# tennisonliu/bayesian-neural-network

Measured on AMD Instinct MI355X. Metric: MC-forward-samples/sec + KL-elements/sec, 784-1200-1200-10 BNN, higher is better.
Workload: dtype bf16

## Files before the change

### bayesian-neural-network_amd/bnn_hip/engine.py

```python
from __future__ import annotations

import os
from typing import List, Optional, Sequence, Tuple

import torch

from . import _lib as L
from . import ops
from .functional import AllReduceSumFn, BBBLinearFn, ElboFn, LayerCall, LRLinearFn, NetCall, NLLFn
from .ops import Predictive
from .runtime import state, take_samples


CAST_INPUT_MIN_SAMPLES = 4
CAST_INPUT_MIN_SAMPLES_LR = 1
LR_SQUARES_MIN_SAMPLES = 7
SPLIT_MIN_SAMPLES = 4
SPLIT_MIN_WEIGHTS = 250_000
SPLIT_MAX_UNITS = 1024

FUSED_ELBO_NODE = True


FINAL_ROWS_MAX_SAMPLES = 16
# ... 464 lines not shown
                self.ws[i] = ops.sample_workspace(S, sp.in_out[0], sp.in_out[1], dev)
        shared0 = self.lr and not self.G > 1 and lr_unit_samples(S, True) == 1
        k3s_first = (self.lr and hid == torch.bfloat16 and len(self.specs) > 1 and self.specs[0].in_out[0] % 8 == 0 and
                     lr_use_split(self.specs[0].in_out[1], S, B, shared0) and not self.G > 1)
        shared0 = shared0 and k3s_first
        self.x16 = (torch.empty(self.x.shape, dtype=torch.bfloat16, device=dev)
                    if (hid == torch.bfloat16 and self.x.dtype == torch.float32 and
                        (self.lib[0] or S >= (CAST_INPUT_MIN_SAMPLES_LR if self.lr else CAST_INPUT_MIN_SAMPLES)) and
                        not k3s_first) else None)
        self.x16_lo = torch.empty(self.x.shape, dtype=torch.bfloat16, device=dev) if (self.x3 and self.x16 is not None) else None
        self.lr_sq = self.lr and (self.x16 is not None or (k3s_first and hid == torch.bfloat16)) and S >= LR_SQUARES_MIN_SAMPLES
        self.x16_sq = torch.empty(self.x.shape, dtype=torch.bfloat16, device=dev) if (self.lr_sq and self.x16 is not None) else None
        self.bufs_sq = [torch.empty(b.shape, dtype=torch.bfloat16, device=dev)
                        if (self.lr_sq and i < len(self.bufs) - 1 and b.dtype == torch.bfloat16) else None for i, b in enumerate(self.bufs)]
        self.split = [ops.split_scratch(S, B, sp.in_out[1], dev)
                      if (not self.lr and hid == torch.bfloat16 and not self.lib[i] and
                          use_split(sp.in_out[0], sp.in_out[1], S, B)) else None
                      for i, sp in enumerate(self.specs)]
        self.lr_split = [ops.lr_split_scratch(lr_unit_samples(S, shared0 and i == 0), B, sp.in_out[1], dev)
                         if (self.lr and hid == torch.bfloat16 and i < len(self.specs) - 1 and
                             lr_use_split(sp.in_out[1], S, B, shared0 and i == 0)) else None
                         for i, sp in enumerate(self.specs)]
        self.wsigma = [torch.empty_like(sp.m.weight_rho.detach())
                      if (not self.lr and hid == torch.bfloat16 and not lb and hoist_sigma(*sp.in_out, S, B)) else None
                      for sp, lb in zip(self.specs, self.lib)]
        self.wfrag = [None] * len(self.specs)
        if self.lr_sq:
            frag_bytes = L.load().bnn_lr_prepare_x3_bytes if self.lr_x3 else L.load().bnn_lr_prepare_bytes
            self.wfrag = [torch.empty(frag_bytes(*sp.in_out) // 4, dtype=torch.float32, device=dev)
                          if (lr_use_prepare(sp.in_out[1], S, B) and not (shared0 and i == 0) and not (self.lr_x3 and i == nl_ - 1)) else None
                          for i, sp in enumerate(self.specs)]
        nl = len(self.specs)
        self.lr_rider = None
        if (self.lr_sq and not self.lr_x3 and self.wfrag[nl - 1] is None and any(w is not None for w in self.wfrag) and
                self.scratch is not None and not wide_nll(self.specs, B) and self.specs[-1].in_out[1] <= 16 and S <= LR_FINAL_ROWS_MAX_SAMPLES):
            self.wfrag[nl - 1] = torch.empty(L.load().bnn_lr_prepare_bytes(*self.specs[-1].in_out) // 4, dtype=torch.float32, device=dev)
        if (self.lr and hid == torch.bfloat16 and nl > 1 and self.wfrag[nl - 1] is None and self.scratch is not None and
                not wide_nll(self.specs, B) and self.specs[-1].in_out[1] <= 16 and S <= 16 and self.lr_split[nl - 2] is not None and
                lr_kslice_expected(*self.specs[-2].in_out, S, B)):
            sp = self.specs[-1]
            self.lr_rider = dict(w_mu=sp.m.weight_mu.detach(), w_rho=sp.m.weight_rho.detach(), b_mu=sp.m.bias_mu.detach(),
                                 b_rho=sp.m.bias_rho.detach(), workspace=self.ws[nl - 1],
                                 w_frag=torch.empty(L.load().bnn_lr_prepare_bytes(*sp.in_out) // 4, dtype=torch.float32, device=dev))
        self.pre_from = presample_from(self.specs, S, B, hid)
        self.rows = self.pre_from >= 0
        self.w_pre, self.b_pre = [None] * len(self.specs), [None] * len(self.specs)
        if self.rows:
            for i in range(self.pre_from + 1, len(self.specs)):
                k_i, n_i = self.specs[i].in_out
                self.w_pre[i] = torch.empty((S, n_i, k_i), dtype=torch.bfloat16, device=dev)
                self.b_pre[i] = torch.empty((S, n_i), dtype=torch.float32, device=dev)
                self.ws[i] = ops.sample_workspace(S, k_i, n_i, dev)
        self.k1b2 = self._k1b2_layers() if state.pieces else [False] * nl
        for i in range(nl - 1):
            if self.k1b2[i] and i == 0 and self.x16 is not None:
                self.x16 = ops.pieces_activation(self.x.shape, dev)
            elif self.k1b2[i] and i > 0 and self.k1b2[i - 1]:
                self.bufs[i - 1] = ops.pieces_activation(self.bufs[i - 1].shape, dev)
        self.wpieces = [ops.param_pieces(sp.in_out[1], sp.in_out[0], dev) if (k and state.param_pieces) else None
                        for sp, k in zip(self.specs, self.k1b2)]
        for w, pc in zip(self.wsigma, self.wpieces):
            if pc is not None:
                w.bnn_param_pieces = pc
        self.graph = None
        self.calls = None
        if capture == "calls":
            rec_stream = self.stream if self.stream is not None else torch.cuda.current_stream()
            with torch.cuda.stream(rec_stream):
                self._enqueue()
            take_samples(self.total_samples)
            torch.cuda.synchronize()
            before = torch.cuda.memory_stats(dev).get("allocation.all.allocated", 0)
            with L.recording() as calls, torch.cuda.stream(rec_stream):
                self._eager()
            take_samples(self.total_samples * self.per_replay)
            torch.cuda.synchronize()
            if torch.cuda.memory_stats(dev).get("allocation.all.allocated", 0) != before:
                raise ops.BnnHipError("GraphedElbo(capture='calls'): the evaluation allocated device memory while it was recorded -- "
                                      "a replay would launch on freed buffers; use capture=True (hipGraph) for this configuration")
            self.calls = list(calls)
        elif capture:
            self._enqueue()
            take_samples(self.total_samples)
            torch.cuda.synchronize()
            side = self.stream if self.stream is not None else torch.cuda.Stream()
            side.wait_stream(torch.cuda.current_stream())
            with torch.cuda.stream(side):
                g = torch.cuda.CUDAGraph()
                with torch.cuda.graph(g, stream=side):
                    self._eager()
            torch.cuda.current_stream().wait_stream(side)
            self.graph = g

    def _enqueue(self):
        math_mode = self.math
        h_sq, h_lo = None, None
        hoist = [i for i, w in enumerate(self.wsigma) if w is not None]
        h = self.x
        if self.x16 is not None or hoist:
            ops.eval_prepare([self.specs[i].m.weight_rho.detach() for i in hoist], [self.wsigma[i] for i in hoist],
                             cast=self.x if self.x16 is not None else None, cast_out=self.x16,
                             cast_out_sq=self.x16_sq, cast_out_lo=self.x16_lo,
                             mus=[self.specs[i].m.weight_mu.detach() for i in hoist], pieces=[self.wpieces[i] for i in hoist])
            if self.x16 is not None:
                h, h_sq, h_lo = self.x16, self.x16_sq, self.x16_lo
        last = len(self.specs) - 1
        if self.lr and any(w is not None for w in self.wfrag):
            jobs = [dict(w_mu=sp.m.weight_mu.detach(), w_rho=sp.m.weight_rho.detach(), b_mu=sp.m.bias_mu.detach(),
                         b_rho=sp.m.bias_rho.detach(), workspace=self.ws[i], out=self.wfrag[i])
                    for i, sp in enumerate(self.specs) if self.wfrag[i] is not None]
            ops.lr_prepare_many(jobs, x3=self.lr_x3)
# ... 26 lines not shown
                if i == last:
                    ops.elbo_finalize(workspaces=self.ws, logits=self.bufs[i], **fin_kw)
            else:
                kw = self._bbb_kw(i, h, h_lo, common)
                if i == last and self.rows:
                    ops.bbb_final_fwd((h, None, None, None, None),
                                      dict(n_samples=self.n_local, prior=sp.m._prior_spec, math_mode=math_mode, relu=sp.relu,
                                           y_dtype=self.bufs[i].dtype, eps_mode=L.EPS_ZERO, want_stats=False, out=self.bufs[i],
                                           w_sampled=self.w_pre[i], b_sampled=self.b_pre[i]),
                                      dict(workspaces=self.ws, **fin_kw))
                elif i == last:
                    ops.bbb_final_fwd((h,) + p, kw, dict(workspaces=self.ws[:last], **fin_kw))
                else:
                    ops.bbb_linear_fwd(h, *p, **kw)
            h, h_lo = self.bufs[i], self.bufs_lo[i]
        if self.lr:
            ops.elbo_finalize(workspaces=self.ws, logits=h, **fin_kw)

    def _common_kw(self, i):
        sp = self.specs[i]
        grp = dict(sample_group=self.group, sample_group_stride=self.samples) if self.G > 1 else {}
        return dict(n_samples=self.n_local, math_mode=self.math, relu=sp.relu, y_dtype=self.bufs[i].dtype,
                    eps_mode=L.EPS_PHILOX, seed=state.seed, layer_id=sp.layer_id, sample_offset=self.lo,
                    sample_counter=self.counter, workspace=self.ws[i], out=self.bufs[i], form=state.form, **grp)

    def _bbb_kw(self, i, h, h_lo, common):
        sp = self.specs[i]
        kw = dict(prior=sp.m._prior_spec, want_stats=True, split_scratch=self.split[i], w_sigma=self.wsigma[i], **common)
        if self.x3:
            kw.update(x_lo=h_lo if h.dtype == torch.bfloat16 else None, out_lo=self.bufs_lo[i])
        if i == self.pre_from and i < len(self.specs) - 1:
            grp = dict(sample_group=self.group, sample_group_stride=self.samples) if self.G > 1 else {}
            kw["rider"] = ops.build_sample_job(
                [dict(w_mu=q.m.weight_mu.detach(), w_rho=q.m.weight_rho.detach(), b_mu=q.m.bias_mu.detach(),
                      b_rho=q.m.bias_rho.detach(), prior=q.m._prior_spec, layer_id=q.layer_id,
                      workspace=self.ws[j], w_out=self.w_pre[j], b_out=self.b_pre[j])
                 for j, q in enumerate(self.specs) if j > i],
                n_samples=self.n_local, seed=state.seed, sample_offset=self.lo, sample_counter=self.counter, **grp)
        return kw

    def _k1b2_layers(self):
        res = [False] * len(self.specs)
        if self.lr or self.math != L.MATH_BF16:
            return res
        h = self.x16 if self.x16 is not None else self.x
        for i, sp in enumerate(self.specs[:-1]):
            if not self.lib[i] and self.wsigma[i] is not None and h.dtype == torch.bfloat16:
                p = tuple(t.detach() for t in (sp.m.weight_mu, sp.m.weight_rho, sp.m.bias_mu, sp.m.bias_rho))
                plan = ops.bbb_plan(h, *p, **self._bbb_kw(i, h, None, self._common_kw(i)))
                res[i] = plan["form"] == L.FORM_GEMM and plan["waves"] == 8
            h = self.bufs[i]
        return res

    def _sample_layer(self, i, grp):
        sp = self.specs[i]
        p = tuple(t.detach() for t in (sp.m.weight_mu, sp.m.weight_rho, sp.m.bias_mu, sp.m.bias_rho))
        ops.bbb_sample_weights([dict(w_mu=p[0], w_rho=p[1], b_mu=p[2], b_rho=p[3], prior=sp.m._prior_spec, layer_id=sp.layer_id,
                                     workspace=self.ws[i], w_out=self.lib_w[i], b_out=self.lib_b[i])],
                               n_samples=self.n_local, seed=state.seed, sample_offset=self.lo, sample_counter=self.counter, **grp)

    def _eager(self):
        for _ in range(self.per_replay):
            self._enqueue()

    def replay(self) -> torch.Tensor:
        if self.calls is not None:
            for fn, args, name in self.calls:
                rc = fn(*args)
                if rc:
                    L.check(rc, name)
            take_samples(self.total_samples * self.per_replay)
            return self.sums
        if self.stream is not None:
            with torch.cuda.stream(self.stream):
                self.graph.replay() if self.graph is not None else self._eager()
        elif self.graph is not None:
            self.graph.replay()
        else:
            self._eager()
        take_samples(self.total_samples * self.per_replay)
        return self.sums

    @property
    def logits(self) -> torch.Tensor:
        return self.bufs[-1]


class GraphedPredict(GraphedElbo):

    def __init__(self, net, x: torch.Tensor, samples: int, capture: bool = True, stream: Optional[torch.cuda.Stream] = None):
        if net.mode != "classification":
            raise ops.BnnHipError("GraphedPredict: the MC-averaged class prediction exists for classification networks")
        xf = net._flat(x)
        self.probs = torch.empty((xf.shape[0], net._specs()[-1].in_out[1]), dtype=torch.float32, device=x.device)
        self.preds = torch.empty(xf.shape[0], dtype=torch.int64, device=x.device)
        super().__init__(net, x, torch.zeros(xf.shape[0], dtype=torch.int64, device=x.device), samples, capture=capture, stream=stream)

    def _enqueue(self):
        super()._enqueue()
        ops.mc_softmax_mean(self.logits, 1.0 / self.samples, out_probs=self.probs, out_preds=self.preds if self.world == 1 else None,
                            want_preds=self.world == 1)

    def replay(self):
        super().replay()
        if self.world > 1:
            import torch.distributed as dist
# ... 92 lines not shown
```

### bayesian-neural-network_amd/bnn_hip/ops.py

```python
from __future__ import annotations

import ctypes as C
import math
from dataclasses import dataclass
from typing import NamedTuple, Optional, Sequence

import torch

from . import _lib as L
from ._lib import BnnHipError


@dataclass(frozen=True)
class PriorSpec:
    mixture: bool = False
    sigma_p: float = 1.0
    pi: float = 0.5
    sigma1: float = 1.0
    sigma2: float = 1.0

    @staticmethod
    def from_init(prior_init: Sequence[float], mixture: bool) -> "PriorSpec":
        if mixture:
            assert len(prior_init) == 3, "Scale Mixture Prior requires three values in prior initialisation"
# ... 20 lines not shown

def _f32c(t: torch.Tensor, name: str) -> torch.Tensor:
    if t.dtype != torch.float32:
        raise BnnHipError(f"{name} must be float32, got {t.dtype}")
    return t if t.is_contiguous() else t.contiguous()


def _ptr(t: Optional[torch.Tensor]) -> Optional[int]:
    return None if t is None else t.data_ptr()


def _dt(t: torch.Tensor) -> int:
    if t.dtype == torch.float32:
        return L.F32
    if t.dtype == torch.bfloat16:
        return L.BF16
    raise BnnHipError(f"activations must be float32 or bfloat16, got {t.dtype}")


def _exact_unless_bf16(math_mode: int) -> int:
    return L.MATH_F32 if math_mode == L.MATH_BF16X3 else math_mode


def pieces_activation(shape, device) -> torch.Tensor:
    shape = tuple(int(d) for d in shape)
    if len(shape) not in (2, 3) or min(shape) < 1:
        raise BnnHipError(f"pieces_activation: shape must be [batch,features] or [rows,batch,features], got {shape}")
    rows = shape[0] if len(shape) == 3 else 1
    t = torch.zeros((rows * ((shape[-2] + 127) // 128), (shape[-1] + 31) // 32, 8, 64, 8), dtype=torch.bfloat16, device=device)
    t.bnn_pieces = shape
    return t


def param_pieces(out_features: int, in_features: int, device) -> torch.Tensor:
    return torch.zeros(((out_features + 15) // 16, (in_features + 31) // 32, 4, 64, 4), dtype=torch.float32, device=device)


def pieces_shape(t: Optional[torch.Tensor]):
    return getattr(t, "bnn_pieces", None) if t is not None else None


def unpiece(t: torch.Tensor) -> torch.Tensor:
    shape = pieces_shape(t)
    rows, B, K = (shape if len(shape) == 3 else (1,) + shape)
    mbs, ks = (B + 127) // 128, (K + 31) // 32
    v = t.view(rows, mbs, ks, 8, 4, 16, 8).permute(0, 1, 3, 5, 2, 4, 6).reshape(rows, mbs * 128, ks * 32)
    return v[:, :B, :K].reshape(shape).contiguous()


def _x3(x: torch.Tensor, n_samples: int, pieces_ok: bool = False):
    shape = pieces_shape(x)
    if shape is not None:
        if not pieces_ok:
            raise BnnHipError("a piece-order activation buffer (ops.pieces_activation) is read by bbb_linear_fwd only")
        if len(shape) == 3 and n_samples % shape[0]:
            raise BnnHipError(f"x has {shape[0]} row blocks, which does not divide {n_samples} samples")
        return x, shape[-2], shape[-1], (n_samples // shape[0] if len(shape) == 3 else 0)
    if x.dim() == 2:
        xs = x if x.is_contiguous() else x.contiguous()
        return xs, x.shape[0], x.shape[1], 0
    if x.dim() == 3:
        if x.shape[0] < 1 or n_samples % x.shape[0]:
            raise BnnHipError(f"x has {x.shape[0]} row blocks, which does not divide {n_samples} samples")
        xs = x if x.is_contiguous() else x.contiguous()
        return xs, x.shape[1], x.shape[2], n_samples // x.shape[0]
    raise BnnHipError(f"x must be [batch,in] or [rows,batch,in], got {tuple(x.shape)}")


def bbb_workspace(n_samples: int, out_features: int, device) -> torch.Tensor:
    nbytes = L.load().bnn_bbb_linear_fwd_workspace_bytes(n_samples, out_features)
    return torch.empty(nbytes // 4, dtype=torch.float32, device=device)


def split_scratch(n_samples: int, batch: int, out_features: int, device) -> torch.Tensor:
    lib = L.load()
    nbytes = lib.bnn_bbb_split_scratch_bytes(n_samples, batch, out_features)
    t = torch.empty((nbytes + 3) // 4, dtype=torch.int32, device=device)
    t[:lib.bnn_bbb_split_scratch_zero_bytes(n_samples, batch, out_features) // 4].zero_()
    return t


_split_cache = {}


def split_scratch_cached(n_samples: int, batch: int, out_features: int, device) -> torch.Tensor:
    if torch.cuda.is_current_stream_capturing():
        return split_scratch(n_samples, batch, out_features, device)
    key = (str(device), torch.cuda.current_stream(device).cuda_stream, n_samples, batch, out_features)
    t = _split_cache.get(key)
    if t is None:
        if len(_split_cache) >= 16:
            _split_cache.clear()
        t = _split_cache[key] = split_scratch(n_samples, batch, out_features, device)
    return t


def final_scratch(n_samples: int, device) -> torch.Tensor:
    nbytes = L.load().bnn_bbb_final_scratch_bytes(n_samples)
    return torch.zeros((nbytes + 3) // 4, dtype=torch.int32, device=device)


def lr_split_scratch(n_samples: int, batch: int, out_features: int, device) -> torch.Tensor:
    lib = L.load()
    nbytes = lib.bnn_lr_split_scratch_bytes(n_samples, batch, out_features)
    t = torch.empty((nbytes + 3) // 4, dtype=torch.int32, device=device)
    t[:lib.bnn_lr_split_scratch_zero_bytes(n_samples, batch, out_features) // 4].zero_()
    return t
# ... 2680 lines not shown
```

### bayesian-neural-network_amd/bnn_hip/runtime.py

```python
from __future__ import annotations

import os
import threading

from . import _lib as L

_lock = threading.Lock()


class _State:
    def __init__(self):
        m = os.environ.get("BNN_HIP_MATH", "bf16").lower()
        self.math = L.MATH_F32 if m in ("f32", "fp32", "float32") else L.MATH_BF16X3 if m in ("bf16x3", "x3") else L.MATH_BF16
        self.seed = int(os.environ.get("BNN_HIP_SEED", "2026"))
        self.host_eps = os.environ.get("BNN_HIP_EPS", "device").lower() == "host"
        self.counter = 0
        self.shard_samples = False
        self.form = L.FORM_AUTO
        self.pieces = os.environ.get("BNN_HIP_PIECES", "1") != "0"
        self.param_pieces = self.pieces and os.environ.get("BNN_HIP_PARAM_PIECES", "1") != "0"
        self.device_counter = None


state = _State()


def set_math(mode: str):
    m = mode.lower()
    if m in ("bf16", "bfloat16"):
        state.math = L.MATH_BF16
    elif m in ("f32", "fp32", "float32"):
        state.math = L.MATH_F32
    elif m in ("bf16x3", "x3"):
        state.math = L.MATH_BF16X3
    else:
        raise ValueError(f"unknown math mode {mode!r}")


def get_math() -> str:
    return {L.MATH_BF16: "bf16", L.MATH_F32: "f32", L.MATH_BF16X3: "bf16x3"}[state.math]


def manual_seed(seed: int, counter: int = 0):
    with _lock:
        state.seed = int(seed) & 0xFFFFFFFFFFFFFFFF
        state.counter = int(counter)


def take_samples(n: int) -> int:
    with _lock:
        first = state.counter
        state.counter = (state.counter + int(n)) & 0xFFFFFFFF
        return first


def set_host_eps(flag: bool):
    state.host_eps = bool(flag)


def shard_samples(flag: bool = True):
    state.shard_samples = bool(flag)
```

### bayesian-neural-network_amd/csrc/bbb_linear.hip

```cpp
#include "bnn_device.h"
#include "bnn_fin.h"
#include "bbb_sample_body.h"
#include "bbb_block_gemm.h"
#include "../../include/bnn_hip.h"
#include <string.h>

namespace bnn {

struct BbbK {
  const void* x;
  long x_sstride;
  const float* w_mu;
  const float* w_rho;
  const float* w_sigma;
  const float* b_mu;
  const float* b_rho;
  const float* eps_w;
  const float* eps_b;
  float* eps_w_dump;
  float* eps_b_dump;
  void* y;
  float4* ws;
  int S, B, K, N;
  __bf16* y16;
// ... 177 lines not shown
        for (int i = 0; i < 4; ++i) o[i] = (__bf16)v[i];
        *reinterpret_cast<bf16x4*>(yp) = o;
      } else {
#pragma unroll
        for (int i = 0; i < 4; ++i)
          if (nb + i < N) yp[i] = (__bf16)v[i];
      }
      if (p.y_lo) {
        __bf16* lp = reinterpret_cast<__bf16*>(p.y_lo) + yoff;
        bf16x4 l;
#pragma unroll
        for (int i = 0; i < 4; ++i) l[i] = (__bf16)(v[i] - (float)(__bf16)v[i]);
        if (vec_ok) {
          *reinterpret_cast<bf16x4*>(lp) = l;
        } else {
#pragma unroll
          for (int i = 0; i < 4; ++i)
            if (nb + i < N) lp[i] = l[i];
        }
      }
    } else {
      float* yp = reinterpret_cast<float*>(p.y) + yoff;
      if (vec_ok) {
        *reinterpret_cast<float4*>(yp) = make_float4(v[0], v[1], v[2], v[3]);
      } else {
#pragma unroll
        for (int i = 0; i < 4; ++i)
          if (nb + i < N) yp[i] = v[i];
      }
      if (p.y16) {
        __bf16* cp = p.y16 + yoff;
        if (vec_ok) {
          bf16x4 o;
#pragma unroll
          for (int i = 0; i < 4; ++i) o[i] = (__bf16)v[i];
          *reinterpret_cast<bf16x4*>(cp) = o;
        } else {
#pragma unroll
          for (int i = 0; i < 4; ++i)
            if (nb + i < N) cp[i] = (__bf16)v[i];
        }
      }
    }
  }
}

struct FinPack : FinTail {
  int ks;
  uint32_t* ks_ticket;
  float4* ks_stats;
  float* ks_tiles;
};

template <int MATH, int XDT, int R, bool ALIGNED, bool FINAL, bool TRANS = false, bool PRE = false, int MT = 8, bool WT = false>
__device__ __forceinline__ bool bbb_fwd_body(const BbbK& p, const FinPack* fp) {
  constexpr int F = 16 / R;
  extern __shared__ __attribute__((aligned(16))) float lds[];
  const int lane = threadIdx.x & 63, wave = threadIdx.x >> 6, nw = blockDim.x >> 6;
  const int r = lane & 15, q = lane >> 4;
  const int c = r / F, f = r % F;
  const int K = p.K, N = p.N, B = p.B;
  const int ntiles = (N + F - 1) / F, mbs = (B + 16 * MT - 1) / (16 * MT);
  int item;
  const int KS = FINAL ? fp->ks : 1;
  if (!xcd_work_item(ntiles * p.S * mbs * KS, item)) return false;
  const int ks = item % KS;
  item /= KS;
  const int nt = item / (p.S * mbs), s = (item / mbs) % p.S, mb = item % mbs;
  const int n = nt * F + f;
  const bool n_ok = n < N;
  const int nc = min(n, N - 1);
  const int m0 = mb * (16 * MT);
  const int mtiles = min(MT, (B - m0 + 15) >> 4);
  const int ssteps = (K + 32 * R - 1) / (32 * R);
  const int spb = (ssteps + KS - 1) / KS;
  const int t_lo = ks * spb, t_hi = min(ssteps, t_lo + spb);
  const uint32_t gs = global_sample(p, s);
  const bool do_stats = p.want_stats && mb == 0;
  const bool do_ls = do_stats && (s == 0 || FINAL);
  const bool do_dump = mb == 0;
  const int gpr = (int)eps_groups_per_row(K);
  const uint32_t wid = eps_tensor_id(p.layer_id, kEpsWeight);
  const char* xs = reinterpret_cast<const char*>(p.x) + (size_t)(s / p.xg) * (size_t)p.x_sstride * (XDT == BNN_F32 ? 4 : 2);
  constexpr bool X3 = MATH == BNN_MATH_BF16X3;
  static_assert(!X3 || (!TRANS && !PRE && !WT), "the split-bf16 mode is a forward sampling form");
  const char* xs_lo = (X3 && XDT == BNN_BF16) ? reinterpret_cast<const char*>(p.x_lo) + (size_t)(s / p.xg) * (size_t)p.x_sstride * 2 : nullptr;

  float* lds_bias = lds + (size_t)nw * MT * 64 * 4;
  float* lds_red = lds_bias + 16;
  f32x4* slab = reinterpret_cast<f32x4*>(lds);

  BNN_STAMP(0);
  BNN_STAMP_RT(8);
  f32x4 acc[MT];
#pragma unroll
  for (int m = 0; m < MT; ++m) acc[m] = f32x4{0.f, 0.f, 0.f, 0.f};
  float s_e2 = 0.f, s_a = 0.f, s_ls = 0.f;
  if (do_stats && item == 0 && ks == 0 && threadIdx.x == 0)
    p.ws[0] = make_float4(__int_as_float(ntiles), 0.f, 0.f, 0.f);

  float mu_n[8], rho_n[8];
  float4 wraw_n = make_float4(0.f, 0.f, 0.f, 0.f);
  auto load_params = [&](int t) {
    const int k = (t * R + c) * 32 + q * 8;
    if (PRE && TRANS) {
      bf16x8 tw;
#pragma unroll
      for (int j = 0; j < 8; ++j) {
        const __bf16 v = p.w_pre[((size_t)s * K + min(k + j, K - 1)) * p.ldw + nc];
        tw[j] = (k + j < K && n_ok) ? v : (__bf16)0.f;
      }
      wraw_n = __builtin_bit_cast(float4, tw);
    } else if (PRE) {
      wraw_n = *reinterpret_cast<const float4*>(p.w_pre + ((size_t)s * N + nc) * K + min(k, K - 8));
    } else if (TRANS) {
#pragma unroll
      for (int j = 0; j < 8; ++j) {
        const size_t woff = (size_t)min(k + j, K - 1) * p.ldw + nc;
        mu_n[j] = p.w_mu[woff];
        rho_n[j] = p.w_rho[woff];
      }
    } else if (ALIGNED) {
      const size_t woff = (size_t)nc * K + min(k, K - 8);
      load8<true>(p.w_mu + woff, 8, mu_n);
      load8<true>(p.w_rho + woff, 8, rho_n);
    } else {
      const int valid = n_ok ? min(8, K - k) : 0;
      const size_t woff = (size_t)n * K + k;
      load8<false>(p.w_mu + woff, valid, mu_n);
      load8<false>(p.w_rho + woff, valid, rho_n);
    }
  };
  if (t_lo + wave < t_hi) load_params(t_lo + wave);
  float bmu_pre = 0.f, brho_pre = 0.f, beps_pre = 0.f;
  if (PRE) {
    if (!TRANS && wave == nw - 1 && lane < F && n_ok && ks == 0 && p.b_pre) bmu_pre = p.b_pre[(size_t)s * N + n];
  } else if (!TRANS && wave == nw - 1 && lane < F && n_ok && ks == 0) {
    bmu_pre = p.b_mu[n];
    brho_pre = p.b_rho[n];
    beps_pre = bias_eps(p, n, s, gs, do_dump);
  }

#pragma nounroll
  for (int t = t_lo + wave; t < t_hi; t += nw) {
    const int k = (t * R + c) * 32 + q * 8;
    const int valid = n_ok ? min(8, K - k) : 0;
    constexpr int FR = (XDT == BNN_F32 || X3) ? 2 : 1;
    constexpr int MC0 = (8 / (R * FR)) < 1 ? 1 : (8 / (R * FR));
    constexpr int MC = MC0 > MT ? MT : MC0;
    float4 xraw[MC * R * FR];
    auto stage = [&](int ch) {
#pragma unroll
      for (int mm = 0; mm < MC; ++mm) {
        const int row = m0 + (ch * MC + mm) * 16 + r;
#pragma unroll
        for (int cc = 0; cc < R; ++cc) {
          const int xk = (t * R + cc) * 32 + q * 8;
          if (ALIGNED) {
            const size_t off = (size_t)min(row, B - 1) * K + min(xk, K - 8);
            if (XDT == BNN_F32) {
              const float4* px = reinterpret_cast<const float4*>(reinterpret_cast<const float*>(xs) + off);
              xraw[(mm * R + cc) * 2 + 0] = px[0];
              xraw[(mm * R + cc) * 2 + 1] = px[1];
            } else if (X3) {
              xraw[(mm * R + cc) * 2 + 0] = *reinterpret_cast<const float4*>(reinterpret_cast<const __bf16*>(xs) + off);
              xraw[(mm * R + cc) * 2 + 1] = *reinterpret_cast<const float4*>(reinterpret_cast<const __bf16*>(xs_lo) + off);
            } else {
              xraw[mm * R + cc] = *reinterpret_cast<const float4*>(reinterpret_cast<const __bf16*>(xs) + off);
            }
          } else {
            const int xvalid = (row < B) ? min(8, K - xk) : 0;
            const size_t off = (size_t)row * K + xk;
            if (XDT == BNN_F32) {
              float v[8];
              load8<false>(reinterpret_cast<const float*>(xs) + off, xvalid, v);
              xraw[(mm * R + cc) * 2 + 0] = make_float4(v[0], v[1], v[2], v[3]);
              xraw[(mm * R + cc) * 2 + 1] = make_float4(v[4], v[5], v[6], v[7]);
            } else {
              bf16x8 vb;
#pragma unroll
              for (int j = 0; j < 8; ++j)
                vb[j] = (j < xvalid) ? (reinterpret_cast<const __bf16*>(xs) + off)[j] : (__bf16)0.0f;
              if (X3) {
                bf16x8 vl;
#pragma unroll
                for (int j = 0; j < 8; ++j)
                  vl[j] = (j < xvalid) ? (reinterpret_cast<const __bf16*>(xs_lo) + off)[j] : (__bf16)0.0f;
                xraw[(mm * R + cc) * 2 + 0] = __builtin_bit_cast(float4, vb);
                xraw[(mm * R + cc) * 2 + 1] = __builtin_bit_cast(float4, vl);
              } else {
                xraw[mm * R + cc] = __builtin_bit_cast(float4, vb);
              }
            }
          }
        }
      }
    };
    stage(0);

    float mu[8], sg[8];
#pragma unroll
    for (int j = 0; j < 8; ++j) {
      mu[j] = mu_n[j];
      sg[j] = rho_n[j];
    }
    const float4 wraw = wraw_n;
// ... 217 lines not shown
        if (p.relu) {
#pragma unroll
          for (int i = 0; i < 4; ++i) v[i] = fmaxf(v[i], 0.f);
        }
        *reinterpret_cast<f32x4*>(fin_lg + brow * 16 + fg * 4) = v;
        if (brow < B) {
          float* yp = reinterpret_cast<float*>(p.y) + ((size_t)s * B + brow) * N + fg * 4;
#pragma unroll
          for (int i = 0; i < 4; ++i)
            if (fg * 4 + i < N) yp[i] = v[i];
        }
      }
      if (threadIdx.x < 64) {
        own0 = wave_sum(q4.x);
        own1 = wave_sum(q4.y);
        own2 = wave_sum(q4.z);
      }
      if (threadIdx.x == 0) {
        p.ws[1 + (size_t)s * ntiles + nt] = make_float4(own0, own1, own2, 0.f);
        fp->ks_ticket[s] = 0u;
      }
    }
    __syncthreads();
    BNN_STAMP(10);
    float a = 0.f, b = 0.f, nll = 0.f;
    const int own_layer = fk.n_layers - 1;
#ifdef BNN_STAMPS
    fin_sample(fk, fp->c, s, T, fin_lg, 16, own_layer, own0, own1, own2, part, a, b, nll, p.dbg ? p.dbg + (size_t)blockIdx.x * 16 : nullptr);
#else
    fin_sample(fk, fp->c, s, T, fin_lg, 16, own_layer, own0, own1, own2, part, a, b, nll);
#endif
    BNN_STAMP(11);
    if (threadIdx.x == 0) {
      fin_store(fk, s, a, b, nll);
      if (fk.S == 1) {
        if (fp->sums) {
          float* so = fp->sums;
          so[0] = a; so[1] = b; so[2] = nll; so[3] = 1.f;
        }
        if (fk.sample_counter) *fk.sample_counter += fk.sample_counter_inc;
      } else if (fp->ticket) {
        fin_samples_meet(fk, fp->sums, fp->ticket);
      }
    }
  }
  return true;
}

template <int MATH, int XDT, int R, bool ALIGNED>
__global__ __launch_bounds__(768) void bbb_fwd_kernel(const BbbK p) {
  bbb_fwd_body<MATH, XDT, R, ALIGNED, false>(p, nullptr);
}

template <int MATH, int XDT>
__global__ __launch_bounds__(768) void bbb_fwd_final_kernel(const BbbK p, const FinPack fp) {
  bbb_fwd_body<MATH, XDT, 1, true, true>(p, &fp);
}

template <int XDT, int R>
__global__ __launch_bounds__(768) void bbb_fwd_rider_kernel(const BbbK p, const SampleK sk, int n_main) {
  if ((int)blockIdx.x >= n_main) {
    extern __shared__ __attribute__((aligned(16))) float lds[];
    sample_block(sk, (int)blockIdx.x - n_main, lds);
    return;
  }
  bbb_fwd_body<BNN_MATH_BF16, XDT, R, true, false>(p, nullptr);
}

struct FinRows {
  const void* x;
  long x_sstride;
  int xg;
  const __bf16* w;
  const float* b;
  float* y;
  int S, B, K, N, relu;
  uint32_t* tickets;
  float* parts;
};

template <bool XF32>
__global__ __launch_bounds__(256) void bbb_final_rows_kernel(const FinRows p, const FinPack fp, const FinLoss tr) {
  __shared__ __attribute__((aligned(16))) f32x4 red[4][64];
  __shared__ float lg[16][17];
  __shared__ __attribute__((aligned(8))) float part[4 * kFinNV];
  const FinK& fk = fp.k;
  const int RB = (p.B + 15) >> 4;
  const int s = (int)blockIdx.x / (RB + 1), rb = (int)blockIdx.x - s * (RB + 1);
  const int lane = threadIdx.x & 63, wave = threadIdx.x >> 6;
  float pub0 = 0.f, pub1 = 0.f;
  int slot = rb;
  if (rb == RB) {
    int T[8];
#pragma unroll
    for (int l = 0; l < 8; ++l) T[l] = (l < fk.n_layers) ? __float_as_int(reinterpret_cast<const float4*>(fk.ws[l])[0].x) : 0;
    float a = 0.f, b = 0.f, nll = 0.f;
    fin_sample(fk, fp.c, s, T, nullptr, 0, -1, 0.f, 0.f, 0.f, part, a, b, nll);
    pub0 = a;
    pub1 = b;
    slot = 8;
  } else {
    const int r = lane & 15, q = lane >> 4;
    const int K = p.K, N = p.N, B = p.B;
    const int row = min(rb * 16 + r, B - 1);
    const size_t xoff = (size_t)(s / p.xg) * (size_t)p.x_sstride + (size_t)row * K;
    const __bf16* xr = reinterpret_cast<const __bf16*>(p.x) + xoff;
    const float* xr32 = reinterpret_cast<const float*>(p.x) + xoff;
    const __bf16* wr = p.w + ((size_t)s * N + min(r, N - 1)) * K;
    const int ksteps = (K + 31) >> 5;
// ... 1377 lines not shown
    if (err != hipSuccess) return (int)err;
  } else {
#define BNN_GO(MATH, XDT, RR, AL)                                                              \
  do {                                                                                         \
    err = allow_big_lds(bbb_fwd_kernel<MATH, XDT, RR, AL>, pl.lds);                            \
    if (err == hipSuccess)                                                                     \
      hipLaunchKernelGGL((bbb_fwd_kernel<MATH, XDT, RR, AL>), grid, block, pl.lds, stream, k); \
  } while (0)
#define BNN_GO_R(MATH, XDT)                                   \
  do {                                                        \
    if (!al) BNN_GO(MATH, XDT, 1, false);                     \
    else if (pl.R == 1) BNN_GO(MATH, XDT, 1, true);           \
    else if (pl.R == 2) BNN_GO(MATH, XDT, 2, true);           \
    else BNN_GO(MATH, XDT, 4, true);                          \
  } while (0)
    if (math == BNN_MATH_BF16) {
      if (xdt == BNN_F32) BNN_GO_R(BNN_MATH_BF16, BNN_F32); else BNN_GO_R(BNN_MATH_BF16, BNN_BF16);
    } else if (math == BNN_MATH_BF16X3) {
      if (xdt == BNN_F32) BNN_GO_R(BNN_MATH_BF16X3, BNN_F32); else BNN_GO_R(BNN_MATH_BF16X3, BNN_BF16);
    } else {
      if (xdt == BNN_F32) BNN_GO_R(BNN_MATH_F32, BNN_F32); else BNN_GO_R(BNN_MATH_F32, BNN_BF16);
    }
#undef BNN_GO
#undef BNN_GO_R
    if (err != hipSuccess) return (int)err;
  }
  err = hipGetLastError();
  if (err != hipSuccess) return (int)err;
  if (a->log_prior || a->log_q) {
    hipLaunchKernelGGL(bbb_layer_scalars_kernel, dim3(a->n_samples), dim3(256), 0, stream, k.ws, K, a->out_features,
                       a->prior, a->log_prior, a->log_q);
    err = hipGetLastError();
    if (err != hipSuccess) return (int)err;
  }
  return BNN_OK;
}

extern "C" int bnn_bbb_linear_fwd(const bnn_bbb_fwd_args* a, void* stream_) {
  return bbb_linear_fwd_impl(a, stream_, false, nullptr, 0);
}

static constexpr int kFinalTicketMaxSamples = 16;
static constexpr int kRowsTicketMaxSamples = 64;

extern "C" size_t bnn_bbb_final_scratch_bytes(int32_t n_samples) {
  return n_samples <= 0 ? 0 : fin_scratch(nullptr, (size_t)n_samples).bytes;
}

extern "C" int bnn_bbb_final_fwd(const bnn_bbb_fwd_args* a, const bnn_finalize_args* f, void* stream_) {
  BbbK k;
  bool al = false;
  int rc = prepare(a, k, al);
  if (rc != BNN_OK) return rc;
  if (a->x_layout || a->y_layout || a->w_pieces) return BNN_ERR_ENUM;
  FinPack fp;
  rc = make_fin(f, fp.k, fp.c);
  if (rc != BNN_OK) return rc;
  const int nl = f->n_layers;
  rc = check_fin_loss(f);
  if (rc != BNN_OK) return rc;
  if (a->w_sampled) {
    const int S = a->n_samples, B = a->batch, N = a->out_features, K = a->in_features;
    const bool rows = a->y_dtype == BNN_F32 && N <= 16 && B <= 128 && S <= 4096 && !f->local_reparam &&
                      nl >= 1 && f->n_samples == S && f->classes == N && f->batch == B && f->logits == a->y && f->nll &&
                      f->scratch && f->scratch_bytes >= bnn_bbb_final_scratch_bytes(S) &&
                      !(reinterpret_cast<uintptr_t>(f->scratch) & 15) &&
                      (S == 1 || f->ticket || (S > kRowsTicketMaxSamples && !f->loss)) && !a->rider &&
                      (N % 4 != 0 || !(reinterpret_cast<uintptr_t>(a->y) & 15));
    if (!rows) {
      rc = bnn_bbb_linear_fwd(a, stream_);
      if (rc == BNN_OK) rc = bnn_elbo_finalize(f, stream_);
      return rc != BNN_OK ? rc : bnn_loss_tail_(f, stream_);
    }
    const FinLoss tr = make_fin_loss(f);
    FinRows fr;
    fr.x = a->x;
    fr.x_sstride = k.x_sstride; fr.xg = k.xg;
    fr.w = k.w_pre; fr.b = k.b_pre;
    fr.y = reinterpret_cast<float*>(a->y);
    fr.S = S; fr.B = B; fr.K = K; fr.N = N; fr.relu = a->relu ? 1 : 0;
    const FinScratch sc = fin_scratch(f->scratch, (size_t)S);
    fr.tickets = sc.tickets;
    fr.parts = sc.stats;
    const bool rows_tail = S > kRowsTicketMaxSamples && !tr.out4;
    fp.sums = f->sums;
    fp.ticket = rows_tail ? nullptr : f->ticket;
    fp.ks = 1; fp.ks_ticket = nullptr; fp.ks_stats = nullptr; fp.ks_tiles = nullptr;
    const int RB = (B + 15) / 16;
    if (a->x_dtype == BNN_BF16)
      hipLaunchKernelGGL(bbb_final_rows_kernel<false>, dim3((unsigned)(S * (RB + 1))), dim3(256), 0, reinterpret_cast<hipStream_t>(stream_),
                         fr, fp, tr);
    else
      hipLaunchKernelGGL(bbb_final_rows_kernel<true>, dim3((unsigned)(S * (RB + 1))), dim3(256), 0, reinterpret_cast<hipStream_t>(stream_),
                         fr, fp, tr);
    const hipError_t e2 = hipGetLastError();
    if (e2 != hipSuccess) return (int)e2;
    return rows_tail ? bnn_elbo_sums_(f, stream_) : (int)BNN_OK;
  }
  const bool fuse = al && a->out_features <= 16 && a->batch <= 128 && a->want_stats && !f->local_reparam && nl >= 1 &&
                    f->layer_workspace[nl - 1] == a->workspace && f->n_samples == a->n_samples &&
                    f->classes == a->out_features && f->batch == a->batch && a->y_dtype == BNN_F32 &&
                    (a->n_samples == 1 || a->n_samples > kFinalTicketMaxSamples || f->ticket != nullptr) && !(a->log_prior || a->log_q) &&
                    a->form == BNN_FORM_AUTO;
  if (!fuse) {
    rc = bnn_bbb_linear_fwd(a, stream_);
    if (rc != BNN_OK) return rc;
    rc = bnn_elbo_finalize(f, stream_);
    return rc != BNN_OK ? rc : bnn_loss_tail_(f, stream_);
  }
  hipStream_t stream = reinterpret_cast<hipStream_t>(stream_);
  fp.sums = f->sums;
  const bool tail_kernel = a->n_samples > kFinalTicketMaxSamples;
  fp.ticket = tail_kernel ? nullptr : f->ticket;
  const int K = a->in_features;
  const int ssteps = (K + 31) / 32;
  int KS = (ssteps + 11) / 12;
  KS = KS > kFinalMaxSlices ? kFinalMaxSlices : KS;
  for (int ks = KS; ks <= kFinalMaxSlices; ++ks) {
    const int per = (ssteps + ks - 1) / ks;
    if (per <= 12 && ((per & 3) == 0 || per < 4)) {
      KS = ks;
      break;
    }
  }
  if ((long)a->n_samples * KS > 128) KS = 1;
  if (KS > 1 && (!f->scratch || f->scratch_bytes < bnn_bbb_final_scratch_bytes(a->n_samples) ||
                 (reinterpret_cast<uintptr_t>(f->scratch) & 15)))
    KS = 1;
  const int spb = (ssteps + KS - 1) / KS;
  int spw = 1;
  while ((spb + spw - 1) / spw > 12) ++spw;
  int nw = (spb + spw - 1) / spw;
  nw = nw < 1 ? 1 : nw;
  fp.ks = KS;
  const FinScratch sc = fin_scratch(f->scratch, (size_t)a->n_samples);
  fp.ks_ticket = sc.tickets;
  fp.ks_stats = reinterpret_cast<float4*>(sc.stats);
  fp.ks_tiles = sc.tiles;
  const long total = (long)a->n_samples * KS;
  hipError_t err = hipSuccess;
  const dim3 grid((unsigned)(((total + 7) / 8) * 8)), block(nw * 64);
  const size_t lds = ((size_t)nw * 8 * 64 * 4 + 16 + 3 * nw + 128 * 16 + kFinMaxWaves * kFinNV) * sizeof(float);
#define BNN_FIN(MATH, XDT)                                                                     \
  do {                                                                                         \
    err = allow_big_lds(bbb_fwd_final_kernel<MATH, XDT>, lds);                                 \
    if (err == hipSuccess)                                                                     \
      hipLaunchKernelGGL((bbb_fwd_final_kernel<MATH, XDT>), grid, block, lds, stream, k, fp);  \
  } while (0)
  if (a->math == BNN_MATH_BF16) {
    if (a->x_dtype == BNN_F32) BNN_FIN(BNN_MATH_BF16, BNN_F32); else BNN_FIN(BNN_MATH_BF16, BNN_BF16);
  } else if (a->math == BNN_MATH_BF16X3) {
    if (a->x_dtype == BNN_F32) BNN_FIN(BNN_MATH_BF16X3, BNN_F32); else BNN_FIN(BNN_MATH_BF16X3, BNN_BF16);
  } else {
    if (a->x_dtype == BNN_F32) BNN_FIN(BNN_MATH_F32, BNN_F32); else BNN_FIN(BNN_MATH_F32, BNN_BF16);
  }
#undef BNN_FIN
  if (err != hipSuccess) return (int)err;
  err = hipGetLastError();
  if (err != hipSuccess) return (int)err;
  rc = tail_kernel ? bnn_elbo_sums_(f, stream_) : (int)BNN_OK;
  return rc != BNN_OK ? rc : bnn_loss_tail_(f, stream_);
}

extern "C" int bnn_bbb_input_grad_(const bnn_bbb_bwd_args* a, const float* gz, void* stream_) {
  hipStream_t stream = reinterpret_cast<hipStream_t>(stream_);
  if (a->w_sampled_t) {
    if (a->math != BNN_MATH_BF16) return BNN_ERR_ENUM;
    bnn_bbb_fwd_args fa{};
    fa.struct_bytes = sizeof(bnn_bbb_fwd_args);
    fa.n_samples = a->n_samples; fa.batch = a->batch;
    fa.in_features = a->out_features;
    fa.out_features = a->in_features;
    const bool g16 = a->gy_bf16 && gz == a->gy;
    fa.x = g16 ? a->gy_bf16 : static_cast<const void*>(gz);
    fa.x_dtype = g16 ? BNN_BF16 : BNN_F32;
    fa.x_per_sample = 1;
    fa.math = BNN_MATH_BF16; fa.eps_mode = BNN_EPS_ZERO;
    fa.y = a->g_x; fa.y_dtype = BNN_F32;
    fa.y_bf16_copy = a->g_x_bf16;
    fa.w_sampled = a->w_sampled_t;
    fa.b_sampled = a->b_mu;
    fa.prior = a->prior;
    return bbb_linear_fwd_impl(&fa, stream_, true, a->gx_relu_mask ? a->x : nullptr,
                               a->x_per_sample ? (long)a->batch * a->in_features : 0);
  }
  BbbK k{};
  k.x = gz;
  k.x_sstride = (long)a->batch * a->out_features;
  k.w_mu = a->w_mu; k.w_rho = a->w_rho; k.b_mu = a->b_mu; k.b_rho = a->b_rho;
  k.w_sigma = nullptr;
  k.eps_w = a->eps_w; k.eps_b = a->eps_b; k.eps_w_dump = nullptr; k.eps_b_dump = nullptr;
  k.y = a->g_x;
  k.ws = nullptr;
  k.S = a->n_samples; k.B = a->batch;
  k.K = a->out_features;
  k.N = a->in_features;
  k.ldw = a->in_features;
  k.mask = a->gx_relu_mask ? a->x : nullptr;
  k.mask_sstride = a->x_per_sample ? (long)a->batch * a->in_features : 0;
  k.w_pre = reinterpret_cast<const __bf16*>(a->w_sampled);
  k.b_pre = nullptr;
  k.eps_mode = a->eps_mode; k.prior_kind = a->prior.kind; k.want_stats = 0; k.relu = 0; k.y_bf16 = 0; k.spb = 1;
// ... 49 lines not shown
```

Before: 509,300.

## Feed piece-order activations into the fused final output-layer kernel

Lets the fused final-layer ELBO kernel read the last hidden activation in the piece (MFMA-tiled) layout, so the preceding hidden layer can write that layout directly. The final kernel then loads x fragments as contiguous float4 per lane instead of gathering rows. This is meant to cut strided global loads and layout shuffling on the output layer. In exchange it adds a kernel template variant, new env gating and extra eligibility checks that return an error if the fused path is not taken.

```diff
diff --git a/bayesian-neural-network_amd/bnn_hip/engine.py b/bayesian-neural-network_amd/bnn_hip/engine.py
--- a/bayesian-neural-network_amd/bnn_hip/engine.py
+++ b/bayesian-neural-network_amd/bnn_hip/engine.py
@@ -540,11 +540,14 @@
                 self.b_pre[i] = torch.empty((S, n_i), dtype=torch.float32, device=dev)
                 self.ws[i] = ops.sample_workspace(S, k_i, n_i, dev)
         self.k1b2 = self._k1b2_layers() if state.pieces else [False] * nl
+        self.k1c = self._k1c_final()
         for i in range(nl - 1):
             if self.k1b2[i] and i == 0 and self.x16 is not None:
                 self.x16 = ops.pieces_activation(self.x.shape, dev)
             elif self.k1b2[i] and i > 0 and self.k1b2[i - 1]:
                 self.bufs[i - 1] = ops.pieces_activation(self.bufs[i - 1].shape, dev)
+        if nl >= 2 and self.k1b2[nl - 2] and self.k1c and state.final_pieces:
+            self.bufs[nl - 2] = ops.pieces_activation(self.bufs[nl - 2].shape, dev)
         self.wpieces = [ops.param_pieces(sp.in_out[1], sp.in_out[0], dev) if (k and state.param_pieces) else None
                         for sp, k in zip(self.specs, self.k1b2)]
         for w, pc in zip(self.wsigma, self.wpieces):
@@ -677,6 +680,13 @@
             h = self.bufs[i]
         return res
 
+    def _k1c_final(self):
+        last = len(self.specs) - 1
+        k_last, n_last = self.specs[last].in_out
+        return (not self.lr and self.math == L.MATH_BF16 and not self.rows and not self.lib[last] and
+                self._common_kw(last)["form"] == L.FORM_AUTO and self.n_local > FINAL_ROWS_MAX_SAMPLES and
+                n_last <= 16 and self.x.shape[-2] <= 128 and k_last % 8 == 0)
+
     def _sample_layer(self, i, grp):
         sp = self.specs[i]
         p = tuple(t.detach() for t in (sp.m.weight_mu, sp.m.weight_rho, sp.m.bias_mu, sp.m.bias_rho))
diff --git a/bayesian-neural-network_amd/bnn_hip/ops.py b/bayesian-neural-network_amd/bnn_hip/ops.py
--- a/bayesian-neural-network_amd/bnn_hip/ops.py
+++ b/bayesian-neural-network_amd/bnn_hip/ops.py
@@ -96,7 +96,7 @@
     shape = pieces_shape(x)
     if shape is not None:
         if not pieces_ok:
-            raise BnnHipError("a piece-order activation buffer (ops.pieces_activation) is read by bbb_linear_fwd only")
+            raise BnnHipError("a piece-order activation buffer (ops.pieces_activation) is read by bbb_linear_fwd / bbb_final_fwd only")
         if len(shape) == 3 and n_samples % shape[0]:
             raise BnnHipError(f"x has {shape[0]} row blocks, which does not divide {n_samples} samples")
         return x, shape[-2], shape[-1], (n_samples // shape[0] if len(shape) == 3 else 0)
diff --git a/bayesian-neural-network_amd/bnn_hip/runtime.py b/bayesian-neural-network_amd/bnn_hip/runtime.py
--- a/bayesian-neural-network_amd/bnn_hip/runtime.py
+++ b/bayesian-neural-network_amd/bnn_hip/runtime.py
@@ -19,6 +19,7 @@
         self.form = L.FORM_AUTO
         self.pieces = os.environ.get("BNN_HIP_PIECES", "1") != "0"
         self.param_pieces = self.pieces and os.environ.get("BNN_HIP_PARAM_PIECES", "1") != "0"
+        self.final_pieces = self.pieces and os.environ.get("BNN_HIP_FINAL_PIECES", "1") != "0"
         self.device_counter = None
 
 
diff --git a/bayesian-neural-network_amd/csrc/bbb_linear.hip b/bayesian-neural-network_amd/csrc/bbb_linear.hip
--- a/bayesian-neural-network_amd/csrc/bbb_linear.hip
+++ b/bayesian-neural-network_amd/csrc/bbb_linear.hip
@@ -253,9 +253,12 @@
   float* ks_tiles;
 };
 
-template <int MATH, int XDT, int R, bool ALIGNED, bool FINAL, bool TRANS = false, bool PRE = false, int MT = 8, bool WT = false>
+template <int MATH, int XDT, int R, bool ALIGNED, bool FINAL, bool TRANS = false, bool PRE = false, int MT = 8, bool WT = false,
+          bool XTL = false>
 __device__ __forceinline__ bool bbb_fwd_body(const BbbK& p, const FinPack* fp) {
   constexpr int F = 16 / R;
+  static_assert(!XTL || (FINAL && R == 1 && ALIGNED && MT == 8 && XDT == BNN_BF16 && MATH == BNN_MATH_BF16),
+                "piece-order x: the fused output layer in bf16 math");
   extern __shared__ __attribute__((aligned(16))) float lds[];
   const int lane = threadIdx.x & 63, wave = threadIdx.x >> 6, nw = blockDim.x >> 6;
   const int r = lane & 15, q = lane >> 4;
@@ -353,6 +356,10 @@
     auto stage = [&](int ch) {
 #pragma unroll
       for (int mm = 0; mm < MC; ++mm) {
+        if constexpr (XTL) {
+          xraw[mm] = *reinterpret_cast<const float4*>(xs + ((size_t)((t * 8 + ch * MC + mm) * 64 + lane)) * 16);
+          continue;
+        }
         const int row = m0 + (ch * MC + mm) * 16 + r;
 #pragma unroll
         for (int cc = 0; cc < R; ++cc) {
@@ -676,9 +683,9 @@
   bbb_fwd_body<MATH, XDT, R, ALIGNED, false>(p, nullptr);
 }
 
-template <int MATH, int XDT>
+template <int MATH, int XDT, bool XTL = false>
 __global__ __launch_bounds__(768) void bbb_fwd_final_kernel(const BbbK p, const FinPack fp) {
-  bbb_fwd_body<MATH, XDT, 1, true, true>(p, &fp);
+  bbb_fwd_body<MATH, XDT, 1, true, true, false, false, 8, false, XTL>(p, &fp);
 }
 
 template <int XDT, int R>
@@ -2162,7 +2169,8 @@
   bool al = false;
   int rc = prepare(a, k, al);
   if (rc != BNN_OK) return rc;
-  if (a->x_layout || a->y_layout || a->w_pieces) return BNN_ERR_ENUM;
+  const bool x_pieces = a->x_layout == BNN_LAYOUT_PIECES;
+  if (a->y_layout || a->w_pieces || (x_pieces && (a->w_sampled || a->math != BNN_MATH_BF16))) return BNN_ERR_ENUM;
   FinPack fp;
   rc = make_fin(f, fp.k, fp.c);
   if (rc != BNN_OK) return rc;
@@ -2212,6 +2220,7 @@
                     f->classes == a->out_features && f->batch == a->batch && a->y_dtype == BNN_F32 &&
                     (a->n_samples == 1 || a->n_samples > kFinalTicketMaxSamples || f->ticket != nullptr) && !(a->log_prior || a->log_q) &&
                     a->form == BNN_FORM_AUTO;
+  if (x_pieces && !fuse) return BNN_ERR_ENUM;
   if (!fuse) {
     rc = bnn_bbb_linear_fwd(a, stream_);
     if (rc != BNN_OK) return rc;
@@ -2224,6 +2233,7 @@
   fp.ticket = tail_kernel ? nullptr : f->ticket;
   const int K = a->in_features;
   const int ssteps = (K + 31) / 32;
+  if (x_pieces) k.x_sstride = a->x_per_sample ? (long)ssteps * 4096 : 0;
   int KS = (ssteps + 11) / 12;
   KS = KS > kFinalMaxSlices ? kFinalMaxSlices : KS;
   for (int ks = KS; ks <= kFinalMaxSlices; ++ks) {
@@ -2257,7 +2267,11 @@
     if (err == hipSuccess)                                                                     \
       hipLaunchKernelGGL((bbb_fwd_final_kernel<MATH, XDT>), grid, block, lds, stream, k, fp);  \
   } while (0)
-  if (a->math == BNN_MATH_BF16) {
+  if (x_pieces) {
+    err = allow_big_lds(bbb_fwd_final_kernel<BNN_MATH_BF16, BNN_BF16, true>, lds);
+    if (err == hipSuccess)
+      hipLaunchKernelGGL((bbb_fwd_final_kernel<BNN_MATH_BF16, BNN_BF16, true>), grid, block, lds, stream, k, fp);
+  } else if (a->math == BNN_MATH_BF16) {
     if (a->x_dtype == BNN_F32) BNN_FIN(BNN_MATH_BF16, BNN_F32); else BNN_FIN(BNN_MATH_BF16, BNN_BF16);
   } else if (a->math == BNN_MATH_BF16X3) {
     if (a->x_dtype == BNN_F32) BNN_FIN(BNN_MATH_BF16X3, BNN_F32); else BNN_FIN(BNN_MATH_BF16X3, BNN_BF16);
```

Measured after the change: 517,300, median of 6. +1.6%, better.
